# 86885974647565434342125458569795756674/torch.distributed.pipeline.sync.Pipe

Measured on AMD Instinct MI355X. Metric: tokens/sec for 12-layer Transformer at PP=N (pipeline-parallel training), higher is better.
Workload: dtype bf16

## Files before the change

mipipe/csrc/kernels/gemm.hip:

```cpp
#include <algorithm>
#include <cstdlib>
#include <type_traits>

#include "common.h"
#include "kernels.h"

namespace mipipe {

namespace {

constexpr int BM = 128, BN = 128, BK = 64;
constexpr int kThreads = 256;
constexpr int kTileBytes = BM * BK * 2;
constexpr int kBufBytes = 2 * kTileBytes;
constexpr int kSmemBytes = 2 * kBufBytes;

typedef __attribute__((ext_vector_type(4))) short s16x4;
typedef __attribute__((ext_vector_type(8))) short s16x8;
typedef __attribute__((address_space(3))) s16x4 lds_s16x4;

__device__ __forceinline__ int kc_off(int r, int c16) { return r * 128 + ((c16 ^ ((r >> 1) & 7)) << 4); }

__device__ __forceinline__ int ic_rk(int r) { return (r & 3) | (((r >> 3) & 1) << 2); }
__device__ __forceinline__ int ic_off(int r, int c8) { return r * 256 + ((c8 ^ (ic_rk(r) << 2)) << 3); }
// ... 72 lines not shown
}

template <bool A_KC, bool B_KC, int EPI, int ACT>
__global__ void __launch_bounds__(kThreads) gemm_kernel(GemmArgs g) {
  extern __shared__ __attribute__((aligned(16))) char smem[];
  const int tid = threadIdx.x;
  const int lane = tid & 63;
  const int wave = tid >> 6;
  const int wm = wave >> 1, wn = wave & 1;

  int tm, tn;
  tile_coords(g.M / BM, g.N / BN, tm, tn);
  const int m0 = tm * BM, n0 = tn * BN;

  const bf16_t* A = reinterpret_cast<const bf16_t*>(g.A);
  const bf16_t* B = reinterpret_cast<const bf16_t*>(g.B);

  f32x4 acc[4][4];
#pragma unroll
  for (int i = 0; i < 4; ++i)
#pragma unroll
    for (int j = 0; j < 4; ++j) acc[i][j] = f32x4{0.f, 0.f, 0.f, 0.f};

  Stager<A_KC> sa;
  Stager<B_KC> sb;
  const int nk = g.K / BK;

  sa.load(A, g.lda, m0, 0, tid);
  sb.load(B, g.ldb, n0, 0, tid);
  sa.store(smem, tid);
  sb.store(smem + kTileBytes, tid);
  __syncthreads();

  for (int kt = 0; kt < nk; ++kt) {
    char* cur = smem + (kt & 1) * kBufBytes;
    const bool more = kt + 1 < nk;
    if (more) {
      sa.load(A, g.lda, m0, (kt + 1) * BK, tid);
      sb.load(B, g.ldb, n0, (kt + 1) * BK, tid);
    }
#pragma unroll
    for (int s = 0; s < 2; ++s) {
      bf16x8 af[4], bfr[4];
#pragma unroll
      for (int t = 0; t < 4; ++t) af[t] = read_frag<A_KC>(cur, wm * 64 + 16 * t, s, lane);
#pragma unroll
      for (int t = 0; t < 4; ++t) bfr[t] = read_frag<B_KC>(cur + kTileBytes, wn * 64 + 16 * t, s, lane);
#pragma unroll
      for (int i = 0; i < 4; ++i)
#pragma unroll
        for (int j = 0; j < 4; ++j) acc[i][j] = __builtin_amdgcn_mfma_f32_16x16x32_bf16(af[i], bfr[j], acc[i][j], 0, 0, 0);
    }
    if (more) {
      char* nxt = smem + ((kt + 1) & 1) * kBufBytes;
      sa.store(nxt, tid);
      sb.store(nxt + kTileBytes, tid);
    }
    __syncthreads();
  }

  const int quad = lane >> 4, col_in = lane & 15;
  const float pscale = g.p > 0.f ? 1.f / (1.f - g.p) : 1.f;
#pragma unroll
  for (int i = 0; i < 4; ++i) {
    const int row0 = m0 + wm * 64 + 16 * i + 4 * quad;
#pragma unroll
    for (int j = 0; j < 4; ++j) {
      const int col = n0 + wn * 64 + 16 * j + col_in;
      f32x4 v = acc[i][j];
      if (EPI == kEpiAccumF32) {
        float* C = reinterpret_cast<float*>(g.C);
#pragma unroll
        for (int r = 0; r < 4; ++r) {
          float* p = C + (int64_t)(row0 + r) * g.ldc + col;
          *p += v[r];
        }
      } else if (EPI == kEpiStoreF32) {
        float* C = reinterpret_cast<float*>(g.C);
#pragma unroll
        for (int r = 0; r < 4; ++r) C[(int64_t)(row0 + r) * g.ldc + col] = v[r];
      } else {
        bf16_t* C = reinterpret_cast<bf16_t*>(g.C);
        const float b = g.bias != nullptr ? bf2f(reinterpret_cast<const bf16_t*>(g.bias)[col]) : 0.f;
        float pre[4], out[4];
#pragma unroll
        for (int r = 0; r < 4; ++r) {
          pre[r] = v[r] + b;
          out[r] = ACT == kActRelu ? fmaxf(pre[r], 0.f) : (ACT == kActGelu ? gelu_f(pre[r]) : pre[r]);
        }
        if (g.p > 0.f) {
          const uint4 w = Philox(g.seed, drop_sub(row0, col, g.N), g.offset).next4();
          const uint32_t ws[4] = {w.x, w.y, w.z, w.w};
#pragma unroll
          for (int r = 0; r < 4; ++r) out[r] = drop_keep(ws[r], col & 1, g.threshold >> 16) ? out[r] * pscale : 0.f;
        }
#pragma unroll
        for (int r = 0; r < 4; ++r) {
          if (g.dact_in != nullptr && g.dact == kActReluBits)
            out[r] *= (reinterpret_cast<const uint8_t*>(g.dact_in)[(int64_t)(row0 + r) * g.ldd + (col >> 3)] >> (col & 7)) & 1
                          ? g.dact_scale : 0.f;
          else if (g.dact_in != nullptr)
            out[r] *= g.dact_scale *
                      dact_f(g.dact, bf2f(reinterpret_cast<const bf16_t*>(g.dact_in)[(int64_t)(row0 + r) * g.ldd + col]));
          if (g.res != nullptr) out[r] += bf2f(reinterpret_cast<const bf16_t*>(g.res)[(int64_t)(row0 + r) * g.ldr + col]);
          C[(int64_t)(row0 + r) * g.ldc + col] = f2bf(out[r]);
          if (g.aux != nullptr)
            reinterpret_cast<bf16_t*>(g.aux)[(int64_t)(row0 + r) * g.ldc + col] =
                f2bf(g.aux_grad ? gelu_grad_f(pre[r]) : pre[r]);
        }
      }
    }
  }
}

namespace big {

constexpr int BM = 256, BN = 256, BK = 64;
constexpr int kThreads = 512;
constexpr int kTileBytes = BM * BK * 2;
constexpr int kSmemBytes = 128 * 260 * 4;

template <bool B_KC, int W>
constexpr int smem_bytes() {
  constexpr int b3 = 2 * (kTileBytes + W * BK * 2) + W * BK * 2;
  return !B_KC && b3 > kSmemBytes ? b3 : kSmemBytes;
}

template <int W>
__device__ __forceinline__ int ic_off_w(int r, int c8) { return r * (2 * W) + ((c8 ^ (ic_rk(r) << 2)) << 3); }

template <bool KC, int W>
__device__ __forceinline__ void stage_offsets(int64_t ld, int i0, int lim, int wave, int lane, uint32_t (&off)[W / 64]) {
  constexpr int NU = W / 64, LPR = W / 8;
#pragma unroll
  for (int u = 0; u < NU; ++u) {
    const int inst = wave * NU + u;
    if (KC) {
      const int row = 8 * inst + (lane >> 3);
      const int c = (lane & 7) ^ ((row >> 1) & 7);
      const int gi = min(i0 + row, lim - 1);
      off[u] = (uint32_t)(((int64_t)gi * ld + 8 * c) * 2);
    } else {
      const int row = (64 / LPR) * inst + lane / LPR;
      const int c16 = (lane % LPR) ^ (ic_rk(row) << 1);
      const int gi = min(i0 + 8 * c16, lim - 8);
      off[u] = (uint32_t)(((int64_t)row * ld + gi) * 2);
    }
  }
}

__device__ __forceinline__ void stage_offsets_halves(int64_t ld, int i0, int lim, int share, int lane,
                                                     uint32_t (&off)[4]) {
  const int half = share >> 2;
#pragma unroll
  for (int u = 0; u < 4; ++u) {
    const int row = 4 * (4 * (share & 3) + u) + (lane >> 4);
    const int c16 = (lane & 15) ^ (ic_rk(row) << 1);
    const int gi = min(i0 + 128 * half + 8 * c16, lim - 8);
    off[u] = (uint32_t)(((int64_t)row * ld + gi) * 2);
  }
}

__device__ __forceinline__ void glds16_saddr(const char* base, uint32_t off, const char* lds_dst) {
  const uint32_t m0 = (uint32_t)(uintptr_t)((__attribute__((address_space(3))) const char*)lds_dst);
  asm volatile(
      "s_mov_b32 m0, %0\n\t"
      "s_nop 0\n\t"
      "global_load_lds_dwordx4 %1, %2"
      :
      : "s"(m0), "v"(off), "s"(base)
      : "memory", "m0");
}

template <int N>
__device__ __forceinline__ void vmcnt_keep() {
  asm volatile("s_waitcnt vmcnt(%0)" ::"n"(N) : "memory");
}

constexpr int kWaitLgkm0 = 0xC07F;

template <int W>
__device__ __forceinline__ void stage_fast(const char* base, const uint32_t (&off)[W / 64], char* tile, int wave) {
  constexpr int NU = W / 64;
#pragma unroll
  for (int u = 0; u < NU; ++u) glds16_saddr(base, off[u], tile + (wave * NU + u) * 1024);
}

struct KCursor {
  const char *a, *b;
  const char *na, *nb;
  int64_t step_a, step_b;
  int seg_k, kl, seg;

  __device__ __forceinline__ void load_next(const GemmArgs& g) {
    const int nx = min(seg + 1, GemmArgs::kMaxSegs - 1);
    na = reinterpret_cast<const char*>(g.a_seg[nx]);
    nb = reinterpret_cast<const char*>(g.b_seg[nx]);
  }
  template <bool A_KC, bool B_KC>
  __device__ __forceinline__ void init(const GemmArgs& g, int kt) {
    const int64_t lda = g.lda, ldb = g.ldb;
    step_a = A_KC ? BK * 2 : BK * lda * 2;
    step_b = B_KC ? BK * 2 : BK * ldb * 2;
    seg_k = g.seg_k;
    kl = kt * BK;
    seg = 0;
    a = na = reinterpret_cast<const char*>(g.A);
    b = nb = reinterpret_cast<const char*>(g.B);
    if (seg_k > 0) {
      seg = kl / seg_k;
      kl -= seg * seg_k;
      a = reinterpret_cast<const char*>(g.a_seg[seg]);
      b = reinterpret_cast<const char*>(g.b_seg[seg]);
      load_next(g);
    }
    a += A_KC ? (int64_t)kl * 2 : (int64_t)kl * lda * 2;
    b += B_KC ? (int64_t)kl * 2 : (int64_t)kl * ldb * 2;
  }
  __device__ __forceinline__ void next(const GemmArgs& g) {
    a += step_a;
    b += step_b;
    kl += BK;
    if (__builtin_expect(kl == seg_k, 0)) {
      kl = 0;
      ++seg;
      a = na;
      b = nb;
      load_next(g);
    }
  }
};

template <bool KC, int W>
__device__ __forceinline__ bf16x8 frag(const char* tile, int ib, int s, int lane) {
  if (KC) {
    const int r = ib + (lane & 15);
    const int c = 4 * s + (lane >> 4);
    return *reinterpret_cast<const bf16x8*>(tile + kc_off(r, c));
  } else {
    const int g = lane >> 4, q = (lane & 15) >> 2, p = lane & 3;
    const int r0 = 32 * s + 8 * g + q;
    const int c8 = (ib >> 2) + p;
    const s16x4 lo = __builtin_amdgcn_ds_read_tr16_b64_v4i16((lds_s16x4*)(tile + ic_off_w<W>(r0, c8)));
    const s16x4 hi = __builtin_amdgcn_ds_read_tr16_b64_v4i16((lds_s16x4*)(tile + ic_off_w<W>(r0 + 4, c8)));
    return __builtin_bit_cast(bf16x8, __builtin_shufflevector(lo, hi, 0, 1, 2, 3, 4, 5, 6, 7));
  }
}

template <int W>
__device__ __forceinline__ uint32_t ic_frag_off(int ib, int lane) {
  const int g = lane >> 4, q = (lane & 15) >> 2, p = lane & 3;
  return (uint32_t)ic_off_w<W>(8 * g + q, (ib >> 2) + p);
}

template <int W>
__device__ __forceinline__ bf16x8 ic_frag_at(uint32_t addr, int imm, int s) {
  const s16x4 lo = __builtin_amdgcn_ds_read_tr16_b64_v4i16((lds_s16x4*)(addr + (uint32_t)(imm + s * 32 * 2 * W)));
  const s16x4 hi =
      __builtin_amdgcn_ds_read_tr16_b64_v4i16((lds_s16x4*)(addr + (uint32_t)(imm + s * 32 * 2 * W + 4 * 2 * W)));
  return __builtin_bit_cast(bf16x8, __builtin_shufflevector(lo, hi, 0, 1, 2, 3, 4, 5, 6, 7));
}

struct EpiParams {
  uint64_t seed, offset;
  int N;
  float p, pscale;
  uint32_t threshold;
  int mask_row0, mask_col0, mask_ld;
};

template <int I, int ACT, int NJ, bool EXTRA>
__device__ __forceinline__ void epi_rows(const EpiParams ep, f32x4 (&acc)[8][NJ], int nrow, int ncol,
                                         const float (&bias)[NJ]) {
  if constexpr (!EXTRA) {
#pragma unroll
    for (int j = 0; j < NJ; ++j)
#pragma unroll
      for (int r = 0; r < 4; ++r) {
        const float pre = acc[I][j][r] + bias[j];
        acc[I][j][r] = ACT == kActRelu ? fmaxf(pre, 0.f) : (ACT == kActGelu ? gelu_f(pre) : pre);
      }
    return;
  }
  const int row0 = nrow + 16 * I;
#pragma unroll
  for (int j = 0; j < NJ; ++j) {
    const int col = ncol + 16 * j;
    const float b = bias[j];
    uint32_t ws[4] = {0xFFFFFFFFu, 0xFFFFFFFFu, 0xFFFFFFFFu, 0xFFFFFFFFu};
    if (ep.p > 0.f) {
      const uint4 w = Philox(ep.seed, drop_sub(row0 + ep.mask_row0, col + ep.mask_col0, ep.mask_ld), ep.offset).next4();
      ws[0] = w.x; ws[1] = w.y; ws[2] = w.z; ws[3] = w.w;
    }
#pragma unroll
    for (int r = 0; r < 4; ++r) {
      const float pre = acc[I][j][r] + b;
      float out = ACT == kActRelu ? fmaxf(pre, 0.f) : (ACT == kActGelu ? gelu_f(pre) : pre);
      if (ep.p > 0.f) out = drop_keep(ws[r], (col + ep.mask_col0) & 1, ep.threshold >> 16) ? out * ep.pscale : 0.f;
      acc[I][j][r] = out;
    }
  }
}

template <int EPI, int W>
__device__ __forceinline__ void staged_store(char* smem, const f32x4 (&acc)[8][W / 64], int wm, int wn, int lane,
                                             int tid, int m0, int n0, int M, int N, int64_t ldc, void* out,
                                             const bf16_t* res, int64_t ldr = 0, const bf16_t* dact_in = nullptr,
                                             int64_t ldd = 0, int dact = 0, float dact_scale = 1.f,
                                             bool trans = false, bool dgelu = false) {
  constexpr int NJ = W / 64, WN = 16 * NJ, kStride = W + 4;
  const int quad = lane >> 4, col_in = lane & 15;
  float* stg = reinterpret_cast<float*>(smem);
#pragma unroll
  for (int pass = 0; pass < 2; ++pass) {
    if (wm == pass) {
#pragma unroll
      for (int i = 0; i < 8; ++i)
#pragma unroll
        for (int j = 0; j < NJ; ++j)
#pragma unroll
          for (int r = 0; r < 4; ++r)
            stg[(16 * i + 4 * quad + r) * kStride + wn * WN + 16 * j + col_in] = acc[i][j][r];
    }
    __syncthreads();
    const int rbase = m0 + pass * 128;
    auto grow = [&](int R) { return rbase + R; };
    if (EPI == kEpiStoreBf16) {
      bf16_t* C = reinterpret_cast<bf16_t*>(out);
      constexpr int CPR = W / 8;
#pragma unroll
      for (int u = 0; u < 128 * CPR / kThreads; ++u) {
        const int idx = tid + u * kThreads;
        const int row = idx / CPR, c8 = idx % CPR;
        if (grow(row) >= M || n0 + 8 * c8 >= N) continue;
        const f32x4 lo = *reinterpret_cast<const f32x4*>(stg + row * kStride + 8 * c8);
        const f32x4 hi = *reinterpret_cast<const f32x4*>(stg + row * kStride + 8 * c8 + 4);
        const int64_t at = (int64_t)grow(row) * ldc + n0 + 8 * c8;
        float v[8] = {lo[0], lo[1], lo[2], lo[3], hi[0], hi[1], hi[2], hi[3]};
        if (dgelu) {
#pragma unroll
          for (int e = 0; e < 8; ++e) v[e] = gelu_grad_f(v[e]);
        }
        if (dact_in != nullptr && dact == kActReluBits) {
          const uint32_t mb =
              reinterpret_cast<const uint8_t*>(dact_in)[(int64_t)grow(row) * ldd + ((n0 + 8 * c8) >> 3)];
#pragma unroll
          for (int e = 0; e < 8; ++e) v[e] *= (mb >> e) & 1 ? dact_scale : 0.f;
        } else if (dact_in != nullptr) {
          const bf16x8 sv = *reinterpret_cast<const bf16x8*>(dact_in + (int64_t)grow(row) * ldd + n0 + 8 * c8);
#pragma unroll
          for (int e = 0; e < 8; ++e) v[e] *= dact_scale * dact_f(dact, (float)sv[e]);
        }
        if (res != nullptr) {
          const bf16x8 rv = *reinterpret_cast<const bf16x8*>(res + (int64_t)grow(row) * ldr + n0 + 8 * c8);
#pragma unroll
          for (int e = 0; e < 8; ++e) v[e] += (float)rv[e];
        }
        bf16x8 o;
#pragma unroll
        for (int e = 0; e < 8; ++e) o[e] = (__bf16)v[e];
        *reinterpret_cast<bf16x8*>(C + at) = o;
      }
    } else if (trans) {
      float* C = reinterpret_cast<float*>(out);
#pragma unroll 4
      for (int u = 0; u < 32 * W / kThreads; ++u) {
        const int idx = tid + u * kThreads;
        const int mq = (idx & 7) + 8 * (idx / (8 * W)), n = (idx >> 3) % W;
        if (grow(4 * mq) >= M || n0 + n >= N) continue;
        const float* sp = stg + 4 * mq * kStride + n;
        const float4 v = make_float4(sp[0], sp[kStride], sp[2 * kStride], sp[3 * kStride]);
        float4* dst = reinterpret_cast<float4*>(C + (int64_t)(n0 + n) * ldc + grow(4 * mq));
        if (EPI == kEpiAccumF32) {
          const float4 o = *dst;
          *dst = make_float4(o.x + v.x, o.y + v.y, o.z + v.z, o.w + v.w);
        } else {
          *dst = v;
        }
      }
    } else {
      float* C = reinterpret_cast<float*>(out);
      constexpr int CPR = W / 4;
#pragma unroll
      for (int u = 0; u < 128 * CPR / kThreads; ++u) {
        const int idx = tid + u * kThreads;
        const int row = idx / CPR, c4 = idx % CPR;
        if (grow(row) >= M || n0 + 4 * c4 >= N) continue;
        const float4 v = *reinterpret_cast<const float4*>(stg + row * kStride + 4 * c4);
        float4* dst = reinterpret_cast<float4*>(C + (int64_t)grow(row) * ldc + n0 + 4 * c4);
        if (EPI == kEpiAccumF32) {
          const float4 o = *dst;
          *dst = make_float4(o.x + v.x, o.y + v.y, o.z + v.z, o.w + v.w);
        } else {
          *dst = v;
        }
      }
    }
    __syncthreads();
  }
}

template <int ACT, int W>
__device__ __forceinline__ void staged_store_act(char* smem, const f32x4 (&acc)[8][W / 64], int wm, int wn,
                                                 int lane, int tid, int m0, int n0, const GemmArgs& g) {
  constexpr int NJ = W / 64, WN = 16 * NJ, kStride = W + 4, CB = W / 8;
  const int quad = lane >> 4, col_in = lane & 15;
  float* stg = reinterpret_cast<float*>(smem);
  bf16_t* C = reinterpret_cast<bf16_t*>(g.C);
  bf16_t* aux = reinterpret_cast<bf16_t*>(g.aux);
  const bf16_t* res = reinterpret_cast<const bf16_t*>(g.res);
  const bf16_t* dact_in = reinterpret_cast<const bf16_t*>(g.dact_in);
  const int64_t ldr = g.ldr > 0 ? g.ldr : g.ldc;
  const bool drop = g.p > 0.f;
  const float pscale = drop ? 1.f / (1.f - g.p) : 1.f;
  const int64_t mask_ld = g.mask_ld > 0 ? g.mask_ld : g.N;
  const uint32_t thr16 = g.threshold >> 16;
#pragma unroll
  for (int pass = 0; pass < 2; ++pass) {
    if (wm == pass) {
#pragma unroll
      for (int i = 0; i < 8; ++i)
#pragma unroll
        for (int j = 0; j < NJ; ++j)
#pragma unroll
          for (int r = 0; r < 4; ++r)
            stg[(16 * i + 4 * quad + r) * kStride + wn * WN + 16 * j + col_in] = acc[i][j][r];
    }
    __syncthreads();
    const int rbase = m0 + pass * 128;
#pragma unroll
    for (int u = 0; u < 32 * CB / kThreads; ++u) {
      const int idx = tid + u * kThreads;
      const int rq = idx / CB, c8 = idx % CB;
      const int col = n0 + 8 * c8;
      const int row0 = rbase + 4 * rq;
      if (col >= g.N || row0 >= g.M) continue;
      uint32_t wd[4][4];
      if (drop) {
        const uint64_t sub = drop_sub(row0 + g.mask_row0, col + g.mask_col0, mask_ld);
#pragma unroll
        for (int e = 0; e < 4; ++e) {
          const uint4 w = Philox(g.seed, sub + e, g.offset).next4();
          wd[e][0] = w.x; wd[e][1] = w.y; wd[e][2] = w.z; wd[e][3] = w.w;
        }
      }
#pragma unroll
      for (int r = 0; r < 4; ++r) {
        const int row = row0 + r;
        if (row >= g.M) break;
        const float* sp = stg + (4 * rq + r) * kStride + 8 * c8;
        const f32x4 lo = *reinterpret_cast<const f32x4*>(sp);
        const f32x4 hi = *reinterpret_cast<const f32x4*>(sp + 4);
        const float pre[8] = {lo[0], lo[1], lo[2], lo[3], hi[0], hi[1], hi[2], hi[3]};
        if (aux != nullptr) {
          bf16x8 a;
#pragma unroll
          for (int e = 0; e < 8; ++e) a[e] = (__bf16)(ACT == kActGelu && g.aux_grad ? gelu_grad_f(pre[e]) : pre[e]);
          *reinterpret_cast<bf16x8*>(aux + (int64_t)row * g.ldc + col) = a;
        }
        float v[8];
#pragma unroll
        for (int e = 0; e < 8; ++e) {
          float o = ACT == kActRelu ? fmaxf(pre[e], 0.f) : (ACT == kActGelu ? gelu_f(pre[e]) : pre[e]);
          if (drop) o = drop_keep(wd[e >> 1][r], e & 1, thr16) ? o * pscale : 0.f;
          v[e] = o;
        }
        if (dact_in != nullptr) {
          const bf16x8 sv = *reinterpret_cast<const bf16x8*>(dact_in + (int64_t)row * g.ldd + col);
#pragma unroll
          for (int e = 0; e < 8; ++e) v[e] *= g.dact_scale * dact_f(g.dact, (float)sv[e]);
        }
        if (res != nullptr) {
          const bf16x8 rv = *reinterpret_cast<const bf16x8*>(res + (int64_t)row * ldr + col);
#pragma unroll
          for (int e = 0; e < 8; ++e) v[e] += (float)rv[e];
        }
        bf16x8 o;
#pragma unroll
        for (int e = 0; e < 8; ++e) o[e] = (__bf16)v[e];
        *reinterpret_cast<bf16x8*>(C + (int64_t)row * g.ldc + col) = o;
        if (g.bits != nullptr) {
          uint32_t mb = 0;
#pragma unroll
          for (int e = 0; e < 8; ++e) mb |= (v[e] != 0.f ? 1u : 0u) << e;
          reinterpret_cast<uint8_t*>(g.bits)[(int64_t)row * g.ldbits + (col >> 3)] = (uint8_t)mb;
        }
      }
    }
    __syncthreads();
  }
}


constexpr int kXEmit = 1, kXColsum = 2;

template <bool A_KC, bool B_KC, int EPI, int ACT, int W, bool EXTRA, int X = 0>
__global__ void __launch_bounds__(kThreads, 1) gemm256_kernel(GemmArgs g) {
  constexpr int NJ = W / 64;
  constexpr int WN = W / 4;
  constexpr int kBuf = kTileBytes + W * BK * 2;
  constexpr bool AH = !A_KC;
  constexpr bool B3 = !B_KC;
  constexpr bool II = AH && B3;
  extern __shared__ __attribute__((aligned(16))) char smem[];
  const int tid = threadIdx.x;
  const int lane = tid & 63;
  const int wave = __builtin_amdgcn_readfirstlane(tid >> 6);
  const int wm = wave >> 2, wn = wave & 3;

  int tm, tn;
  tile_coords((g.M + BM - 1) / BM, (g.N + W - 1) / W, tm, tn, g.group_m);
  tm = __builtin_amdgcn_readfirstlane(tm);
  tn = __builtin_amdgcn_readfirstlane(tn);
  const int m0 = tm * BM, n0 = tn * W;
  f32x4 acc[8][NJ];
#pragma unroll
  for (int i = 0; i < 8; ++i)
#pragma unroll
    for (int j = 0; j < NJ; ++j) acc[i][j] = f32x4{0.f, 0.f, 0.f, 0.f};

  const bool rsum = g.rowsum != nullptr && tn < 16 && !A_KC;
  float rs[4] = {0.f, 0.f, 0.f, 0.f};
  auto rowsum_read = [&](const char* tile, s16x4& v) {
    if (rsum && wm == 0) {
      const int r = tid >> 2, c8 = 4 * tn + (tid & 3);
      v = *reinterpret_cast<const s16x4*>(
          AH ? tile + (tn >> 3) * (kTileBytes / 2) + ic_off_w<128>(r, c8 & 31) : tile + ic_off_w<256>(r, c8));
    }
  };
  auto rowsum_add = [&](const s16x4& v) {
    if (rsum && wm == 0) {
#pragma unroll
      for (int e = 0; e < 4; ++e) rs[e] += __uint_as_float((uint32_t)(uint16_t)v[e] << 16);
    }
  };
  const int tiles_m = (g.M + BM - 1) / BM;
  const int cm_log = __builtin_amdgcn_readfirstlane(2 * tiles_m * 16 >= W ? 0 : 2 * tiles_m * 32 >= W ? 1
                                                    : 2 * tiles_m * 64 >= W ? 2 : 3);
  const int csl = tm + tiles_m * wm;
  const bool csum = X == kXColsum && !B_KC && g.colsum != nullptr && csl < (W / 16 >> cm_log);
  float cs[4] = {0.f, 0.f, 0.f, 0.f};
  auto colsum_step = [&](const char* btile) {
    if (csum) {
      const int t = tid & 255;
      const int q = t & ((4 << cm_log) - 1), r0 = t >> (2 + cm_log);
      for (int j = 0; j < (1 << cm_log); ++j) {
        const s16x4 v = *reinterpret_cast<const s16x4*>(
            btile + ic_off_w<W>(r0 + (j << (6 - cm_log)), (4 << cm_log) * csl + q));
#pragma unroll
        for (int e = 0; e < 4; ++e) cs[e] += __uint_as_float((uint32_t)(uint16_t)v[e] << 16);
      }
    }
  };
  const int ntn = (g.N + W - 1) / W;
  const int ewb = __builtin_amdgcn_readfirstlane((4 * wave) % ntn);
  auto emit_reads = [&](const char* atile, int j, s16x4& a, s16x4& b) {
    const int q = (lane & 15) >> 2, p = lane & 3, gq = lane >> 4;
    const int c16 = 2 * gq + (p >> 1);
    const int r = 8 * (4 * wave + j) + q;
    const int lo = r * 128 + ((c16 ^ ((r >> 1) & 7)) << 4) + 8 * (p & 1);
    const int hi = (r + 4) * 128 + ((c16 ^ (((r + 4) >> 1) & 7)) << 4) + 8 * (p & 1);
    a = __builtin_amdgcn_ds_read_tr16_b64_v4i16((lds_s16x4*)(atile + lo));
    b = __builtin_amdgcn_ds_read_tr16_b64_v4i16((lds_s16x4*)(atile + hi));
  };
  bf16_t* const at_out = X == kXEmit ? reinterpret_cast<bf16_t*>(g.at) : nullptr;
  const int64_t ldat = X == kXEmit ? g.ldat : 0;
  const int M = g.M;
  auto emit_store = [&](int kt, int j, const s16x4& a, const s16x4& b) {
    const int rb = 4 * wave + j;
    bf16_t* at = at_out + (int64_t)(kt * BK + 16 * (lane >> 4) + (lane & 15)) * ldat + m0 + 8 * rb;
    if (m0 + 8 * rb < M) *reinterpret_cast<s16x8*>(at) = __builtin_shufflevector(a, b, 0, 1, 2, 3, 4, 5, 6, 7);
  };
  int kt0 = 0, nk = g.K / BK;
  if (g.k_splits > 1) {
    const int total = nk;
    kt0 = (int)blockIdx.y * total / g.k_splits;
    nk = ((int)blockIdx.y + 1) * total / g.k_splits - kt0;
  }
  const int shA = wave ^ 4;
  const int shB = B_KC ? 2 * wn + (wm == 0 ? 1 : 0) : wave;
  uint32_t offA[4], offB[NJ];
  if constexpr (AH) stage_offsets_halves(g.lda, m0, g.M, shA, lane, offA);
  else stage_offsets<A_KC, 256>(g.lda, m0, g.M, shA, lane, offA);
  stage_offsets<B_KC, W>(g.ldb, n0, g.N, shB, lane, offB);
  constexpr int NB = W / 64;
  constexpr int NA = 4;
  auto abuf = [&](int i) { return II ? smem + i * kTileBytes : smem + i * kBuf; };
  auto bslot = [&](int s) {
    if (II) return smem + 2 * kTileBytes + s * (W * BK * 2);
    return s == 2 ? smem + 2 * kBuf : smem + s * kBuf + kTileBytes;
  };
  KCursor kc;
  kc.init<A_KC, B_KC>(g, kt0);
  stage_fast<256>(kc.a, offA, abuf(0), shA);
  stage_fast<W>(kc.b, offB, bslot(0), shB);
  kc.next(g);
  if (wm == 1 && nk > 1) {
    stage_fast<256>(kc.a, offA, abuf(1), shA);
    stage_fast<W>(kc.b, offB, bslot(1), shB);
    kc.next(g);
  }

  if (wm == 1 && nk > 1) vmcnt_keep<NA + NB>();
  else asm volatile("s_waitcnt vmcnt(0)" ::: "memory");
  __builtin_amdgcn_s_barrier();
  if (wm == 1) __builtin_amdgcn_s_barrier();
  bf16x8 af[8][2], bq[NJ][2];
  int ekt = kt0 % ntn;
  int bs = 0;
  if constexpr (II) {
    const uint32_t lds0 = (uint32_t)(uintptr_t)((__attribute__((address_space(3))) const char*)smem);
    uint32_t aaddr[8], baddr[NJ];
#pragma unroll
    for (int ii = 0; ii < 8; ++ii) aaddr[ii] = lds0 + wm * (kTileBytes / 2) + ic_frag_off<128>(16 * ii, lane);
#pragma unroll
    for (int j = 0; j < NJ; ++j) baddr[j] = ic_frag_off<W>(wn * WN + 16 * j, lane);
    auto k_tile = [&](const int u, auto parity) {
      constexpr int P = decltype(parity)::value;
      char* cur = abuf(P);
      char* nxt = abuf(P ^ 1);
      char* bcur = bslot(bs);
#pragma unroll
      for (int ii = 0; ii < 8; ++ii)
#pragma unroll
        for (int s = 0; s < 2; ++s) af[ii][s] = ic_frag_at<128>(aaddr[ii], P * kTileBytes, s);
      const uint32_t bcur0 = (uint32_t)(uintptr_t)((__attribute__((address_space(3))) const char*)bcur);
#pragma unroll
      for (int j = 0; j < NJ; ++j) {
        const uint32_t ba = bcur0 + baddr[j];
#pragma unroll
        for (int s = 0; s < 2; ++s) bq[j][s] = ic_frag_at<W>(ba, 0, s);
      }
      s16x4 rv;
      rowsum_read(cur, rv);
      const int ahead = wm == 0 ? 1 : 2;
      if (u + ahead < nk) {
        stage_fast<256>(kc.a, offA, wm == 0 ? nxt : cur, shA);
        int bn = bs + ahead;
        if (bn >= 3) bn -= 3;
        stage_fast<W>(kc.b, offB, bslot(bn), shB);
        kc.next(g);
      }
      bs = bs == 2 ? 0 : bs + 1;
      if (wm == 1) {
        if (u + 2 < nk) vmcnt_keep<NA + NB>();
        else asm volatile("s_waitcnt vmcnt(0)" ::: "memory");
      }
      __builtin_amdgcn_s_waitcnt(kWaitLgkm0);
      rowsum_add(rv);
      __builtin_amdgcn_sched_barrier(0);
      __builtin_amdgcn_s_barrier();
      __builtin_amdgcn_sched_barrier(0);
      __builtin_amdgcn_s_setprio(1);
#pragma unroll
      for (int s = 0; s < 2; ++s)
#pragma unroll
        for (int ii = 0; ii < 8; ++ii)
#pragma unroll
          for (int j = 0; j < NJ; ++j)
            acc[ii][j] = __builtin_amdgcn_mfma_f32_16x16x32_bf16(af[ii][s], bq[j][s], acc[ii][j], 0, 0, 0);
      __builtin_amdgcn_s_setprio(0);
      if (wm == 0) asm volatile("s_waitcnt vmcnt(0)" ::: "memory");
      __builtin_amdgcn_sched_barrier(0);
      __builtin_amdgcn_s_barrier();
      __builtin_amdgcn_sched_barrier(0);
    };
    for (int u = 0; u < nk; u += 2) {
      k_tile(u, std::integral_constant<int, 0>{});
      if (u + 1 < nk) k_tile(u + 1, std::integral_constant<int, 1>{});
    }
  }
  for (int u = 0; !II && u < nk; ++u) {
    char* cur = smem + (u & 1) * kBuf;
    char* nxt = smem + ((u + 1) & 1) * kBuf;
    char* bcur = B3 ? bslot(bs) : cur + kTileBytes;
    int ej = -1;
    if (X == kXEmit && A_KC) {
      int e = ewb + ekt;
      while (e >= ntn) e -= ntn;
      ej = tn - e;
      if (ej < 0) ej += ntn;
      if (ntn < 4) {
        for (int j = ej; j < 4; j += ntn) {
          s16x4 a, b;
          emit_reads(cur, j, a, b);
          emit_store(kt0 + u, j, a, b);
        }
        ej = -1;
      } else if (ej > 3) {
        ej = -1;
      }
    }
    s16x4 ea, eb;
    if (X == kXEmit && A_KC && ej >= 0) emit_reads(cur, ej, ea, eb);
#pragma unroll
    for (int ii = 0; ii < 8; ++ii)
#pragma unroll
      for (int s = 0; s < 2; ++s)
        af[ii][s] = AH ? frag<false, 128>(cur + wm * (kTileBytes / 2), 16 * ii, s, lane)
                       : frag<A_KC, 256>(cur, wm * 128 + 16 * ii, s, lane);
#pragma unroll
    for (int j = 0; j < NJ; ++j)
#pragma unroll
      for (int s = 0; s < 2; ++s) bq[j][s] = frag<B_KC, W>(bcur, wn * WN + 16 * j, s, lane);
    s16x4 rv;
    rowsum_read(cur, rv);
    if (X == kXEmit && A_KC && ej >= 0) emit_store(kt0 + u, ej, ea, eb);
    ekt = ekt + 1 == ntn ? 0 : ekt + 1;
    const int ahead = wm == 0 ? 1 : 2;
    if (u + ahead < nk) {
      char* dst = wm == 0 ? nxt : cur;
      stage_fast<256>(kc.a, offA, dst, shA);
      int bn = bs + ahead;
      if (bn >= 3) bn -= 3;
      stage_fast<W>(kc.b, offB, B3 ? bslot(bn) : dst + kTileBytes, shB);
      kc.next(g);
    }
    bs = bs == 2 ? 0 : bs + 1;
    colsum_step(bcur);
    if (wm == 1) {
      if (u + 2 < nk) vmcnt_keep<NA + NB>();
      else asm volatile("s_waitcnt vmcnt(0)" ::: "memory");
    }
    __builtin_amdgcn_s_waitcnt(kWaitLgkm0);
    rowsum_add(rv);
    __builtin_amdgcn_sched_barrier(0);
    __builtin_amdgcn_s_barrier();
    __builtin_amdgcn_sched_barrier(0);
    __builtin_amdgcn_s_setprio(1);
#pragma unroll
    for (int s = 0; s < 2; ++s)
#pragma unroll
      for (int ii = 0; ii < 8; ++ii)
#pragma unroll
        for (int j = 0; j < NJ; ++j)
          acc[ii][j] = __builtin_amdgcn_mfma_f32_16x16x32_bf16(af[ii][s], bq[j][s], acc[ii][j], 0, 0, 0);
    __builtin_amdgcn_s_setprio(0);
    if (wm == 0) asm volatile("s_waitcnt vmcnt(0)" ::: "memory");
    __builtin_amdgcn_sched_barrier(0);
    __builtin_amdgcn_s_barrier();
    __builtin_amdgcn_sched_barrier(0);
  }
  if (wm == 0) __builtin_amdgcn_s_barrier();

  if (rsum) {
    __syncthreads();
    float* red = reinterpret_cast<float*>(smem);
    if (wm == 0) {
#pragma unroll
      for (int e = 0; e < 4; ++e)
#pragma unroll
        for (int o = 4; o < 64; o <<= 1) rs[e] += __shfl_xor(rs[e], o, 64);
      if (lane < 4)
#pragma unroll
        for (int e = 0; e < 4; ++e) red[wave * 16 + 4 * lane + e] = rs[e];
    }
    __syncthreads();
    if (tid < 16) {
      const float v = red[tid] + red[16 + tid] + red[32 + tid] + red[48 + tid];
      const int row = m0 + 16 * tn + tid;
      if (row < g.M) g.rowsum[row] += v;
    }
  }
  if (X == kXColsum && g.colsum != nullptr) {
    __syncthreads();
    const int sw = 16 << cm_log;
    float* red = reinterpret_cast<float*>(smem) + 64;
#pragma unroll
    for (int e = 0; e < 4; ++e)
      for (int o = 4 << cm_log; o < 64; o <<= 1) cs[e] += __shfl_xor(cs[e], o, 64);
    if (lane < (4 << cm_log))
#pragma unroll
      for (int e = 0; e < 4; ++e) red[wave * sw + 4 * lane + e] = cs[e];
    __syncthreads();
    if (tid < 2 * sw) {
      const int gq = tid >> (4 + cm_log), c = tid & (sw - 1);
      const int sl = tm + tiles_m * gq;
      float v = 0.f;
#pragma unroll
      for (int w = 0; w < 4; ++w) v += red[(4 * gq + w) * sw + c];
      const int col = n0 + sw * sl + c;
      if (sl < (W / 16 >> cm_log) && col < g.N) {
        if (g.k_splits > 1) g.colsum[(int64_t)blockIdx.y * g.N + col] = v;
        else g.colsum[col] += v;
      }
    }
  }
  const int quad = lane >> 4, col_in = lane & 15;
  __syncthreads();
  if (EPI == kEpiStoreBf16 && EXTRA) {
    const int ncol = n0 + wn * WN + col_in;
    if (g.bias != nullptr) {
#pragma unroll
      for (int j = 0; j < NJ; ++j) {
        const float b = ncol + 16 * j < g.N ? bf2f(reinterpret_cast<const bf16_t*>(g.bias)[ncol + 16 * j]) : 0.f;
#pragma unroll
        for (int i = 0; i < 8; ++i) acc[i][j] += b;
      }
    }
    staged_store_act<ACT, W>(smem, acc, wm, wn, lane, tid, m0, n0, g);
    return;
  }
  if (EPI == kEpiStoreBf16 && (ACT != kActNone || g.bias != nullptr)) {
    const int ncol = n0 + wn * WN + col_in, nrow = m0 + wm * 128 + 4 * quad;
    const float pscale = g.p > 0.f ? 1.f / (1.f - g.p) : 1.f;
    const EpiParams ep{g.seed, g.offset, g.N, g.p, pscale, g.threshold, g.mask_row0, g.mask_col0,
                       g.mask_ld > 0 ? g.mask_ld : g.N};
    float bias[NJ];
#pragma unroll
    for (int j = 0; j < NJ; ++j)
      bias[j] = (g.bias != nullptr && ncol + 16 * j < g.N) ? bf2f(reinterpret_cast<const bf16_t*>(g.bias)[ncol + 16 * j]) : 0.f;
    epi_rows<0, ACT, NJ, EXTRA>(ep, acc, nrow, ncol, bias);
    epi_rows<1, ACT, NJ, EXTRA>(ep, acc, nrow, ncol, bias);
    epi_rows<2, ACT, NJ, EXTRA>(ep, acc, nrow, ncol, bias);
    epi_rows<3, ACT, NJ, EXTRA>(ep, acc, nrow, ncol, bias);
    epi_rows<4, ACT, NJ, EXTRA>(ep, acc, nrow, ncol, bias);
    epi_rows<5, ACT, NJ, EXTRA>(ep, acc, nrow, ncol, bias);
    epi_rows<6, ACT, NJ, EXTRA>(ep, acc, nrow, ncol, bias);
    epi_rows<7, ACT, NJ, EXTRA>(ep, acc, nrow, ncol, bias);
  }
  void* out = EPI == kEpiStoreBf16 ? g.C
                                   : reinterpret_cast<void*>(reinterpret_cast<float*>(g.C) +
                                                             (int64_t)blockIdx.y * g.M * g.ldc);
  if (EPI == kEpiStoreBf16 && g.dact_in != nullptr)
    staged_store<EPI, W>(smem, acc, wm, wn, lane, tid, m0, n0, g.M, g.N, g.ldc, out,
                         reinterpret_cast<const bf16_t*>(g.res), g.ldr, reinterpret_cast<const bf16_t*>(g.dact_in),
                         g.ldd, g.dact, g.dact_scale);
  else if (EPI != kEpiStoreBf16 && g.trans_c && g.k_splits <= 1)
    staged_store<EPI, W>(smem, acc, wm, wn, lane, tid, m0, n0, g.M, g.N, g.ldc, out, nullptr, 0, nullptr, 0, 0, 1.f,
                         true);
  else
    staged_store<EPI, W>(smem, acc, wm, wn, lane, tid, m0, n0, g.M, g.N, g.ldc, out,
                         EPI == kEpiStoreBf16 ? reinterpret_cast<const bf16_t*>(g.res) : nullptr, g.ldr);
}

}

int big_tiles(const GemmArgs& g, int w) { return ((g.M + big::BM - 1) / big::BM) * ((g.N + w - 1) / w); }

bool use_big(const GemmArgs& g) {
  return g.round_chunk || g.seg_k > 0 || g.at != nullptr || g.trans_c || g.colsum != nullptr || g.rowsum != nullptr ||
         g.M % BM != 0 || g.N % BN != 0 || big_tiles(g, 256) >= 128;
}

int g_gemm_width = -1;
int g_gemm_rounds = -1;

int big_width(const GemmArgs& g) {
  if (g_gemm_width < 0) {
    const char* e = getenv("MIPIPE_GEMM_W");
    g_gemm_width = e ? atoi(e) : 0;
  }
  if (g_gemm_width == 128 || g_gemm_width == 256) return g_gemm_width;
  if (g.width == 128 || g.width == 256) return g.width;
  if (g.k_splits > 1) return 256;
  const int r256 = (big_tiles(g, 256) + 255) / 256, r128 = (big_tiles(g, 128) + 255) / 256;
  return 0.75 * r128 < 1.0 * r256 ? 128 : 256;
}

template <bool A_KC, bool B_KC, int EPI, int ACT, int W, bool EXTRA, int X = 0>
void launch_big(const GemmArgs& g, hipStream_t s) {
  constexpr int smem = big::smem_bytes<B_KC, W>();
  static bool attr_set = false;
  if (!attr_set) {
    (void)hipFuncSetAttribute(
        reinterpret_cast<const void*>(&big::gemm256_kernel<A_KC, B_KC, EPI, ACT, W, EXTRA, X>),
        hipFuncAttributeMaxDynamicSharedMemorySize, smem);
    attr_set = true;
  }
  hipLaunchKernelGGL((big::gemm256_kernel<A_KC, B_KC, EPI, ACT, W, EXTRA, X>), dim3(big_tiles(g, W), g.k_splits),
                     dim3(big::kThreads), smem, s, g);
}

template <bool A_KC, bool B_KC, int EPI, int ACT, bool EXTRA>
void launch_big_w(const GemmArgs& g, hipStream_t s) {
  const bool narrow = big_width(g) == 128;
  if constexpr (A_KC && B_KC && EPI == kEpiStoreBf16 && !(ACT == kActGelu && EXTRA)) {
    if (g.at != nullptr) {
      if (narrow) launch_big<A_KC, B_KC, EPI, ACT, 128, EXTRA, big::kXEmit>(g, s);
      else launch_big<A_KC, B_KC, EPI, ACT, 256, EXTRA, big::kXEmit>(g, s);
      return;
    }
  }
  if constexpr (A_KC && !B_KC && EPI != kEpiStoreBf16 && !EXTRA) {
    if (g.colsum != nullptr) {
      if (narrow) launch_big<A_KC, B_KC, EPI, ACT, 128, EXTRA, big::kXColsum>(g, s);
      else launch_big<A_KC, B_KC, EPI, ACT, 256, EXTRA, big::kXColsum>(g, s);
      return;
    }
  }
  if (narrow) launch_big<A_KC, B_KC, EPI, ACT, 128, EXTRA>(g, s);
  else launch_big<A_KC, B_KC, EPI, ACT, 256, EXTRA>(g, s);
}

int g_gemm_group = -1;

template <bool A_KC, bool B_KC, int EPI, int ACT>
void launch(const GemmArgs& gi, hipStream_t s) {
  if (g_gemm_group < 0) {
    const char* e = getenv("MIPIPE_GEMM_G");
    g_gemm_group = e ? atoi(e) : 0;
  }
  GemmArgs g = gi;
  if (g_gemm_group > 0) g.group_m = g_gemm_group;
  if (use_big(g)) {
    if constexpr (EPI == kEpiStoreBf16) {
      if (g.p > 0.f || g.aux != nullptr) {
        launch_big_w<A_KC, B_KC, EPI, ACT, true>(g, s);
        return;
      }
    }
    launch_big_w<A_KC, B_KC, EPI, ACT, false>(g, s);
    return;
  }
  const int blocks = (g.M / BM) * (g.N / BN);
  hipLaunchKernelGGL((gemm_kernel<A_KC, B_KC, EPI, ACT>), dim3(blocks), dim3(kThreads), kSmemBytes, s, g);
}

__global__ void __launch_bounds__(256) splitk_reduce_kernel(const float* __restrict__ ws, int splits, int M, int N,
                                                            int64_t ldc, const bf16_t* __restrict__ res, int64_t ldr,
                                                            bf16_t* __restrict__ C) {
  const int64_t chunks = (int64_t)M * (N / 8);
  const int64_t c = (int64_t)blockIdx.x * blockDim.x + threadIdx.x;
  if (c >= chunks) return;
  const int row = (int)(c / (N / 8)), col = (int)(c % (N / 8)) * 8;
  const int64_t at = (int64_t)row * N + col;
  f32x4 lo = *reinterpret_cast<const f32x4*>(ws + at);
  f32x4 hi = *reinterpret_cast<const f32x4*>(ws + at + 4);
  for (int s = 1; s < splits; ++s) {
    lo += *reinterpret_cast<const f32x4*>(ws + (int64_t)s * M * N + at);
    hi += *reinterpret_cast<const f32x4*>(ws + (int64_t)s * M * N + at + 4);
  }
  float v[8] = {lo[0], lo[1], lo[2], lo[3], hi[0], hi[1], hi[2], hi[3]};
  const int64_t out = (int64_t)row * ldc + col;
  if (res != nullptr) {
    const bf16x8 r = *reinterpret_cast<const bf16x8*>(res + (int64_t)row * ldr + col);
#pragma unroll
    for (int e = 0; e < 8; ++e) v[e] += (float)r[e];
  }
  bf16x8 o;
#pragma unroll
  for (int e = 0; e < 8; ++e) o[e] = (__bf16)v[e];
  *reinterpret_cast<bf16x8*>(C + out) = o;
}

__global__ void __launch_bounds__(256) splitk_reduce_f32_kernel(const float* __restrict__ ws, int splits, int M, int N,
                                                                int64_t ldc, bool accumulate, bool trans,
                                                                float* __restrict__ C) {
  const int64_t c = (int64_t)blockIdx.x * blockDim.x + threadIdx.x;
  if (trans) {
    if (c >= (int64_t)(M / 4) * N) return;
    const int m = (int)(c / N) * 4, n = (int)(c % N);
    f32x4 v = {0.f, 0.f, 0.f, 0.f};
    for (int s = 0; s < splits; ++s) {
      const float* p = ws + (int64_t)s * M * N + (int64_t)m * N + n;
      v += f32x4{p[0], p[N], p[2 * (int64_t)N], p[3 * (int64_t)N]};
    }
    f32x4* dst = reinterpret_cast<f32x4*>(C + (int64_t)n * ldc + m);
    if (accumulate) v += *dst;
    *dst = v;
    return;
  }
  const int64_t chunks = (int64_t)M * (N / 4);
  if (c >= chunks) return;
  const int row = (int)(c / (N / 4)), col = (int)(c % (N / 4)) * 4;
  const int64_t at = (int64_t)row * N + col;
  f32x4 v = *reinterpret_cast<const f32x4*>(ws + at);
  for (int s = 1; s < splits; ++s) v += *reinterpret_cast<const f32x4*>(ws + (int64_t)s * M * N + at);
  f32x4* dst = reinterpret_cast<f32x4*>(C + (int64_t)row * ldc + col);
  if (accumulate) v += *dst;
  *dst = v;
}

__global__ void __launch_bounds__(256) colsum_splits_kernel(const float* __restrict__ ws, int splits, int N,
                                                            float* __restrict__ colsum) {
  const int n = blockIdx.x * blockDim.x + threadIdx.x;
  if (n >= N) return;
  float v = 0.f;
  for (int s = 0; s < splits; ++s) v += ws[(int64_t)s * N + n];
  colsum[n] += v;
}

int g_gemm_splitk = -1;

template <bool A_KC, bool B_KC, int EPI>
void launch_act(const GemmArgs& g, hipStream_t s) {
  switch (g.act) {
    case kActRelu: launch<A_KC, B_KC, EPI, kActRelu>(g, s); break;
    case kActGelu: launch<A_KC, B_KC, EPI, kActGelu>(g, s); break;
    default: launch<A_KC, B_KC, EPI, kActNone>(g, s); break;
  }
}

}

void gemm_set_width(int w) { g_gemm_width = w; }
void gemm_set_rounds(int on) { g_gemm_rounds = on; }
void gemm_set_splitk(int n) { g_gemm_splitk = n; }

bool gemm_rowsum_ok(const GemmArgs& g) {
  return !g.a_kc && (g.epi == kEpiAccumF32 || g.epi == kEpiStoreF32) && use_big(g) && gemm_splitk_factor(g) <= 1 &&
         (g.N + big_width(g) - 1) / big_width(g) >= 16;
}

bool gemm_bits_ok(const GemmArgs& g) {
  return g.epi == kEpiStoreBf16 && g.act == kActRelu && g.p > 0.f && g.k_splits <= 1 && g.N % 8 == 0 && use_big(g);
}

bool gemm_emit_ok(int act, float p, bool aux) { return !(act == kActGelu && (p > 0.f || aux)); }

bool gemm_colsum_ok(const GemmArgs& g) {
  if (g.b_kc || !g.a_kc || !(g.epi == kEpiAccumF32 || g.epi == kEpiStoreF32)) return false;
  GemmArgs b = g;
  b.k_splits = gemm_splitk_factor(g);
  const int w = big_width(b);
  return 2 * ((g.M + big::BM - 1) / big::BM) * 128 >= w;
}

bool gemm_supported(int64_t M, int64_t N, int64_t K) {
  return M >= 8 && N >= 8 && K > 0 && M % 8 == 0 && N % 8 == 0 && K % BK == 0 && M < (1LL << 30) &&
         N < (1LL << 30) && M * K < (1LL << 31) && N * K < (1LL << 31);
}

int gemm_splitk_factor(const GemmArgs& g) {
  if (g_gemm_splitk < 0) {
    const char* e = getenv("MIPIPE_GEMM_SPLITK");
    g_gemm_splitk = e ? atoi(e) : 1;
  }
  if (g_gemm_splitk == 0) return 1;
  const bool plain_bf16 = g.epi == kEpiStoreBf16 && g.act == kActNone && g.bias == nullptr && g.p <= 0.f &&
                          g.aux == nullptr && g.dact_in == nullptr;
  const bool f32_out = g.epi == kEpiAccumF32 || g.epi == kEpiStoreF32;
  if (!(plain_bf16 || f32_out) || !use_big(g) || g.K < 8192) return 1;
  const int tiles = big_tiles(g, 256);
  const int kt = g.K / BK;
  if (g_gemm_splitk >= 2) return std::max(1, std::min(g_gemm_splitk, kt / 16));
  const double t_tile = 2.0 * 256 * 256 * (double)g.K / 4.5e12;
  const double mn = (double)g.M * g.N;
  int best = 1;
  double best_t = (double)((tiles + 255) / 256) * t_tile;
  for (int sp = 2; sp <= 8 && kt / sp >= 16; ++sp) {
    const double t = (double)((tiles * sp + 255) / 256) * t_tile / sp + (2.0 * sp + 1.0) * 4.0 * mn / 4.0e12;
    if (t < 0.97 * best_t) {
      best = sp;
      best_t = t;
    }
  }
  return best;
}


static const char* byte_off(const void* p, int64_t bytes) {
  return p == nullptr ? nullptr : reinterpret_cast<const char*>(p) + bytes;
}

template <typename F>
bool launch_by_rounds(const GemmArgs& g, F&& run) {
  if (g_gemm_rounds < 0) {
    const char* e = getenv("MIPIPE_GEMM_ROUNDS");
    g_gemm_rounds = e ? atoi(e) : 1;
  }
  if (g_gemm_rounds == 0 || g.k_splits > 1 || !use_big(g) || big_width(g) != 256) return false;
  if (g_gemm_rounds == 1 && g.K < 4096) return false;
  const int tm = (g.M + 255) / 256, tn = (g.N + 255) / 256;
  if (tm * tn <= 256 || (tm * tn) % 256 == 0 || (tm * tn) % 256 > 128) return false;
  const bool along_n = tn >= tm;
  if (along_n && g.rowsum != nullptr) return false;
  if (!along_n && g.colsum != nullptr) return false;
  const int other = along_n ? tm : tn, along = along_n ? tn : tm;
  const int per = 256 / other;
  if (per < 1 || (along + per - 1) / per > 16) return false;
  const int cbytes = g.epi == kEpiStoreBf16 ? 2 : 4;
  for (int t0 = 0; t0 < along; t0 += per) {
    GemmArgs c = g;
    c.round_chunk = true;
    c.width = 256;
    const int lo = t0 * 256, hi = std::min((t0 + per) * 256, along_n ? g.N : g.M);
    c.mask_ld = g.mask_ld > 0 ? g.mask_ld : g.N;
    if (along_n) {
      c.N = hi - lo;
      c.mask_col0 = g.mask_col0 + lo;
      const int64_t boff = (g.b_kc ? (int64_t)lo * g.ldb : (int64_t)lo) * 2;
      c.B = byte_off(g.B, boff);
      for (int i = 0; i < GemmArgs::kMaxSegs; ++i) c.b_seg[i] = byte_off(g.b_seg[i], boff);
      c.C = const_cast<char*>(byte_off(g.C, (g.trans_c ? (int64_t)lo * g.ldc : (int64_t)lo) * cbytes));
      if (g.colsum != nullptr) c.colsum = g.colsum + lo;
      if (t0 > 0) c.at = nullptr;
      c.bias = byte_off(g.bias, (int64_t)lo * 2);
      c.aux = const_cast<char*>(byte_off(g.aux, (int64_t)lo * 2));
      c.res = byte_off(g.res, (int64_t)lo * 2);
      c.dact_in = byte_off(g.dact_in, g.dact == kActReluBits ? (int64_t)lo / 8 : (int64_t)lo * 2);
      c.bits = const_cast<char*>(byte_off(g.bits, (int64_t)lo / 8));
    } else {
      c.M = hi - lo;
      c.mask_row0 = g.mask_row0 + lo;
      if (g.rowsum != nullptr) c.rowsum = g.rowsum + lo;
      const int64_t aoff = (g.a_kc ? (int64_t)lo * g.lda : (int64_t)lo) * 2;
      c.A = byte_off(g.A, aoff);
      for (int i = 0; i < GemmArgs::kMaxSegs; ++i) c.a_seg[i] = byte_off(g.a_seg[i], aoff);
      c.C = const_cast<char*>(byte_off(g.C, (g.trans_c ? (int64_t)lo : (int64_t)lo * g.ldc) * cbytes));
      c.at = const_cast<char*>(byte_off(g.at, (int64_t)lo * 2));
      c.aux = const_cast<char*>(byte_off(g.aux, (int64_t)lo * g.ldc * 2));
      c.res = byte_off(g.res, (int64_t)lo * g.ldr * 2);
      c.dact_in = byte_off(g.dact_in, (int64_t)lo * g.ldd * (g.dact == kActReluBits ? 1 : 2));
      c.bits = const_cast<char*>(byte_off(g.bits, (int64_t)lo * g.ldbits));
    }
    run(c);
  }
  return true;
}

void gemm_bf16(const GemmArgs& gi, hipStream_t s) {
  GemmArgs g = gi;
  g.threshold = dropout_threshold(g.p);
  if (g.ldr == 0) g.ldr = g.ldc;
  if (g.ldd == 0) g.ldd = g.ldc;
  if (g.k_splits > 1) {
    GemmArgs p = g;
    p.epi = kEpiStoreF32;
    p.C = g.ws;
    p.ldc = g.N;
    p.res = nullptr;
    p.trans_c = false;
    p.rowsum = nullptr;
    p.colsum = g.colsum != nullptr ? g.colsum_ws : nullptr;
    if (p.a_kc && p.b_kc) launch<true, true, kEpiStoreF32, kActNone>(p, s);
    else if (p.a_kc && !p.b_kc) launch<true, false, kEpiStoreF32, kActNone>(p, s);
    else if (!p.a_kc && !p.b_kc) launch<false, false, kEpiStoreF32, kActNone>(p, s);
    else launch<false, true, kEpiStoreF32, kActNone>(p, s);
    if (g.epi == kEpiStoreBf16) {
      const int64_t chunks = (int64_t)g.M * (g.N / 8);
      hipLaunchKernelGGL(splitk_reduce_kernel, dim3((unsigned)((chunks + 255) / 256)), dim3(256), 0, s, g.ws,
                         g.k_splits, g.M, g.N, g.ldc, reinterpret_cast<const bf16_t*>(g.res), g.ldr,
                         reinterpret_cast<bf16_t*>(g.C));
    } else {
      const int64_t chunks = (int64_t)g.M * (g.N / 4);
// ... 32 lines not shown
```

Measured before the change: 152,800.

## Prefetch residual and activation side inputs in GEMM epilogue, specialize store paths

Specializes the bf16 staged-store epilogue by side-input type (none, residual, relu bits, activation, both) and by whether the tile touches a matrix edge. For residual-only or bits-only cases it issues the global loads for both passes before the LDS staging and barrier, so their latency overlaps the accumulator spill. The activation-fused store loads residual and activation rows ahead of the dropout and activation math. Edge handling uses clamped addresses, and interior tiles skip the bounds checks. In exchange the templates hold more registers (side-input arrays kept across passes), there are more kernel instantiations, and the unused dgelu parameter is removed.

Result: no change. 154,100, median of 6 (+0.9%).

```diff
diff --git a/mipipe/csrc/kernels/gemm.hip b/mipipe/csrc/kernels/gemm.hip
--- a/mipipe/csrc/kernels/gemm.hip
+++ b/mipipe/csrc/kernels/gemm.hip
@@ -398,15 +398,48 @@
   }
 }
 
-template <int EPI, int W>
+constexpr int kSideNone = 0, kSideRes = 1, kSideBits = 2, kSideAct = 3, kSideAny = 4;
+
+template <int EPI, int W, int SIDE = kSideNone, bool EDGE = true>
 __device__ __forceinline__ void staged_store(char* smem, const f32x4 (&acc)[8][W / 64], int wm, int wn, int lane,
                                              int tid, int m0, int n0, int M, int N, int64_t ldc, void* out,
                                              const bf16_t* res, int64_t ldr = 0, const bf16_t* dact_in = nullptr,
                                              int64_t ldd = 0, int dact = 0, float dact_scale = 1.f,
-                                             bool trans = false, bool dgelu = false) {
+                                             bool trans = false) {
   constexpr int NJ = W / 64, WN = 16 * NJ, kStride = W + 4;
+  constexpr int CPR = W / 8, NU = 128 * CPR / kThreads, RS = kThreads / CPR;
+  constexpr bool kAhead = SIDE == kSideRes || SIDE == kSideBits;
+  constexpr int NB = SIDE == kSideAny && NU > 4 ? NU / 2 : NU;
   const int quad = lane >> 4, col_in = lane & 15;
   float* stg = reinterpret_cast<float*>(smem);
+  const int row_t = tid / CPR, col = n0 + 8 * (tid % CPR);
+  u32x4 rv[2][NU], sv[NU];
+  uint32_t mb[2][NU];
+  const bool bits = SIDE == kSideBits || (SIDE == kSideAny && dact == kActReluBits);
+  auto fetch = [&](int pass, int b) {
+    if (EPI != kEpiStoreBf16 || SIDE == kSideNone) return;
+    const int h = kAhead ? pass : 0;
+    const int row = m0 + pass * 128 + row_t;
+    auto at = [&](int u, int64_t ld, int shift) {
+      if (EDGE) return (int64_t)min(row + u * RS, M - 1) * ld + (min(col, N - 8) >> shift);
+      return (int64_t)row * ld + (col >> shift) + (int64_t)(u * RS) * ld;
+    };
+    if (SIDE == kSideRes || SIDE == kSideAny) {
+#pragma unroll
+      for (int u = b; u < b + NB; ++u) rv[h][u] = *reinterpret_cast<const u32x4*>(res + at(u, ldr, 0));
+    }
+    if (bits) {
+#pragma unroll
+      for (int u = b; u < b + NB; ++u) mb[h][u] = reinterpret_cast<const uint8_t*>(dact_in)[at(u, ldd, 3)];
+    } else if (SIDE == kSideAct || SIDE == kSideAny) {
+#pragma unroll
+      for (int u = b; u < b + NB; ++u) sv[u] = *reinterpret_cast<const u32x4*>(dact_in + at(u, ldd, 0));
+    }
+  };
+  if (kAhead) {
+    fetch(0, 0);
+    fetch(1, 0);
+  }
 #pragma unroll
   for (int pass = 0; pass < 2; ++pass) {
     if (wm == pass) {
@@ -418,44 +451,39 @@
           for (int r = 0; r < 4; ++r)
             stg[(16 * i + 4 * quad + r) * kStride + wn * WN + 16 * j + col_in] = acc[i][j][r];
     }
+    if (!kAhead) fetch(pass, 0);
     __syncthreads();
     const int rbase = m0 + pass * 128;
     auto grow = [&](int R) { return rbase + R; };
     if (EPI == kEpiStoreBf16) {
-      bf16_t* C = reinterpret_cast<bf16_t*>(out);
-      constexpr int CPR = W / 8;
-#pragma unroll
-      for (int u = 0; u < 128 * CPR / kThreads; ++u) {
-        const int idx = tid + u * kThreads;
-        const int row = idx / CPR, c8 = idx % CPR;
-        if (grow(row) >= M || n0 + 8 * c8 >= N) continue;
-        const f32x4 lo = *reinterpret_cast<const f32x4*>(stg + row * kStride + 8 * c8);
-        const f32x4 hi = *reinterpret_cast<const f32x4*>(stg + row * kStride + 8 * c8 + 4);
-        const int64_t at = (int64_t)grow(row) * ldc + n0 + 8 * c8;
-        float v[8] = {lo[0], lo[1], lo[2], lo[3], hi[0], hi[1], hi[2], hi[3]};
-        if (dgelu) {
-#pragma unroll
-          for (int e = 0; e < 8; ++e) v[e] = gelu_grad_f(v[e]);
+      bf16_t* C = reinterpret_cast<bf16_t*>(out) + (int64_t)grow(row_t) * ldc + col;
+      const int h = kAhead ? pass : 0;
+#pragma unroll
+      for (int u = 0; u < NU; ++u) {
+        if (u == NB) fetch(pass, NB);
+        const int row = row_t + u * RS;
+        if (!EDGE || (grow(row) < M && col < N)) {
+          const f32x4 lo = *reinterpret_cast<const f32x4*>(stg + row * kStride + (col - n0));
+          const f32x4 hi = *reinterpret_cast<const f32x4*>(stg + row * kStride + (col - n0) + 4);
+          float v[8] = {lo[0], lo[1], lo[2], lo[3], hi[0], hi[1], hi[2], hi[3]};
+          if (bits) {
+#pragma unroll
+            for (int e = 0; e < 8; ++e) v[e] *= (mb[h][u] >> e) & 1 ? dact_scale : 0.f;
+          } else if (SIDE == kSideAct || SIDE == kSideAny) {
+            const bf16x8 s8 = __builtin_bit_cast(bf16x8, sv[u]);
+#pragma unroll
+            for (int e = 0; e < 8; ++e) v[e] *= dact_scale * dact_f(dact, (float)s8[e]);
+          }
+          if (SIDE == kSideRes || SIDE == kSideAny) {
+            const bf16x8 r8 = __builtin_bit_cast(bf16x8, rv[h][u]);
+#pragma unroll
+            for (int e = 0; e < 8; ++e) v[e] += (float)r8[e];
+          }
+          bf16x8 o;
+#pragma unroll
+          for (int e = 0; e < 8; ++e) o[e] = (__bf16)v[e];
+          *reinterpret_cast<bf16x8*>(C + (int64_t)(u * RS) * ldc) = o;
         }
-        if (dact_in != nullptr && dact == kActReluBits) {
-          const uint32_t mb =
-              reinterpret_cast<const uint8_t*>(dact_in)[(int64_t)grow(row) * ldd + ((n0 + 8 * c8) >> 3)];
-#pragma unroll
-          for (int e = 0; e < 8; ++e) v[e] *= (mb >> e) & 1 ? dact_scale : 0.f;
-        } else if (dact_in != nullptr) {
-          const bf16x8 sv = *reinterpret_cast<const bf16x8*>(dact_in + (int64_t)grow(row) * ldd + n0 + 8 * c8);
-#pragma unroll
-          for (int e = 0; e < 8; ++e) v[e] *= dact_scale * dact_f(dact, (float)sv[e]);
-        }
-        if (res != nullptr) {
-          const bf16x8 rv = *reinterpret_cast<const bf16x8*>(res + (int64_t)grow(row) * ldr + n0 + 8 * c8);
-#pragma unroll
-          for (int e = 0; e < 8; ++e) v[e] += (float)rv[e];
-        }
-        bf16x8 o;
-#pragma unroll
-        for (int e = 0; e < 8; ++e) o[e] = (__bf16)v[e];
-        *reinterpret_cast<bf16x8*>(C + at) = o;
       }
     } else if (trans) {
       float* C = reinterpret_cast<float*>(out);
@@ -500,13 +528,15 @@
 __device__ __forceinline__ void staged_store_act(char* smem, const f32x4 (&acc)[8][W / 64], int wm, int wn,
                                                  int lane, int tid, int m0, int n0, const GemmArgs& g) {
   constexpr int NJ = W / 64, WN = 16 * NJ, kStride = W + 4, CB = W / 8;
+  constexpr int NB = 32 * CB / kThreads;
   const int quad = lane >> 4, col_in = lane & 15;
   float* stg = reinterpret_cast<float*>(smem);
   bf16_t* C = reinterpret_cast<bf16_t*>(g.C);
   bf16_t* aux = reinterpret_cast<bf16_t*>(g.aux);
   const bf16_t* res = reinterpret_cast<const bf16_t*>(g.res);
   const bf16_t* dact_in = reinterpret_cast<const bf16_t*>(g.dact_in);
-  const int64_t ldr = g.ldr > 0 ? g.ldr : g.ldc;
+  const int64_t ldr = g.ldr > 0 ? g.ldr : g.ldc, ldd = g.ldd;
+  const int M = g.M, colc = min(n0 + 8 * (tid % CB), g.N - 8);
   const bool drop = g.p > 0.f;
   const float pscale = drop ? 1.f / (1.f - g.p) : 1.f;
   const int64_t mask_ld = g.mask_ld > 0 ? g.mask_ld : g.N;
@@ -525,11 +555,22 @@
     __syncthreads();
     const int rbase = m0 + pass * 128;
 #pragma unroll
-    for (int u = 0; u < 32 * CB / kThreads; ++u) {
+    for (int u = 0; u < NB; ++u) {
       const int idx = tid + u * kThreads;
       const int rq = idx / CB, c8 = idx % CB;
       const int col = n0 + 8 * c8;
       const int row0 = rbase + 4 * rq;
+      u32x4 rv[4], sv[4];
+      if (res != nullptr) {
+#pragma unroll
+        for (int r = 0; r < 4; ++r)
+          rv[r] = *reinterpret_cast<const u32x4*>(res + (int64_t)min(row0 + r, M - 1) * ldr + colc);
+      }
+      if (dact_in != nullptr) {
+#pragma unroll
+        for (int r = 0; r < 4; ++r)
+          sv[r] = *reinterpret_cast<const u32x4*>(dact_in + (int64_t)min(row0 + r, M - 1) * ldd + colc);
+      }
       if (col >= g.N || row0 >= g.M) continue;
       uint32_t wd[4][4];
       if (drop) {
@@ -562,14 +603,14 @@
           v[e] = o;
         }
         if (dact_in != nullptr) {
-          const bf16x8 sv = *reinterpret_cast<const bf16x8*>(dact_in + (int64_t)row * g.ldd + col);
-#pragma unroll
-          for (int e = 0; e < 8; ++e) v[e] *= g.dact_scale * dact_f(g.dact, (float)sv[e]);
+          const bf16x8 s8 = __builtin_bit_cast(bf16x8, sv[r]);
+#pragma unroll
+          for (int e = 0; e < 8; ++e) v[e] *= g.dact_scale * dact_f(g.dact, (float)s8[e]);
         }
         if (res != nullptr) {
-          const bf16x8 rv = *reinterpret_cast<const bf16x8*>(res + (int64_t)row * ldr + col);
-#pragma unroll
-          for (int e = 0; e < 8; ++e) v[e] += (float)rv[e];
+          const bf16x8 r8 = __builtin_bit_cast(bf16x8, rv[r]);
+#pragma unroll
+          for (int e = 0; e < 8; ++e) v[e] += (float)r8[e];
         }
         bf16x8 o;
 #pragma unroll
@@ -918,16 +959,38 @@
   void* out = EPI == kEpiStoreBf16 ? g.C
                                    : reinterpret_cast<void*>(reinterpret_cast<float*>(g.C) +
                                                              (int64_t)blockIdx.y * g.M * g.ldc);
-  if (EPI == kEpiStoreBf16 && g.dact_in != nullptr)
-    staged_store<EPI, W>(smem, acc, wm, wn, lane, tid, m0, n0, g.M, g.N, g.ldc, out,
-                         reinterpret_cast<const bf16_t*>(g.res), g.ldr, reinterpret_cast<const bf16_t*>(g.dact_in),
-                         g.ldd, g.dact, g.dact_scale);
-  else if (EPI != kEpiStoreBf16 && g.trans_c && g.k_splits <= 1)
+  if constexpr (EPI == kEpiStoreBf16) {
+    const bf16_t* res = reinterpret_cast<const bf16_t*>(g.res);
+    const bf16_t* dact_in = reinterpret_cast<const bf16_t*>(g.dact_in);
+    const int side = dact_in != nullptr
+                         ? (res != nullptr ? kSideAny : (g.dact == kActReluBits ? kSideBits : kSideAct))
+                         : (res != nullptr ? kSideRes : kSideNone);
+    const bool edge = m0 + BM > g.M || n0 + W > g.N;
+    const int lane_e = __builtin_amdgcn_mbcnt_hi(~0u, __builtin_amdgcn_mbcnt_lo(~0u, 0u));
+    const int tid_e = wave * 64 + lane_e;
+#define MIPIPE_STORE_BF16(SIDE, EDGE)                                                                          \
+  staged_store<EPI, W, SIDE, EDGE>(smem, acc, wm, wn, lane_e, tid_e, m0, n0, g.M, g.N, g.ldc, out, res, g.ldr, dact_in, \
+                                   g.ldd, g.dact, g.dact_scale)
+    if (edge) {
+      if (side == kSideNone) MIPIPE_STORE_BF16(kSideNone, true);
+      else if (side == kSideRes) MIPIPE_STORE_BF16(kSideRes, true);
+      else if (side == kSideBits) MIPIPE_STORE_BF16(kSideBits, true);
+      else if (side == kSideAct) MIPIPE_STORE_BF16(kSideAct, true);
+      else MIPIPE_STORE_BF16(kSideAny, true);
+    } else {
+      if (side == kSideNone) MIPIPE_STORE_BF16(kSideNone, false);
+      else if (side == kSideRes) MIPIPE_STORE_BF16(kSideRes, false);
+      else if (side == kSideBits) MIPIPE_STORE_BF16(kSideBits, false);
+      else if (side == kSideAct) MIPIPE_STORE_BF16(kSideAct, false);
+      else MIPIPE_STORE_BF16(kSideAny, false);
+    }
+#undef MIPIPE_STORE_BF16
+  } else if (g.trans_c && g.k_splits <= 1) {
     staged_store<EPI, W>(smem, acc, wm, wn, lane, tid, m0, n0, g.M, g.N, g.ldc, out, nullptr, 0, nullptr, 0, 0, 1.f,
                          true);
-  else
-    staged_store<EPI, W>(smem, acc, wm, wn, lane, tid, m0, n0, g.M, g.N, g.ldc, out,
-                         EPI == kEpiStoreBf16 ? reinterpret_cast<const bf16_t*>(g.res) : nullptr, g.ldr);
+  } else {
+    staged_store<EPI, W>(smem, acc, wm, wn, lane, tid, m0, n0, g.M, g.N, g.ldc, out, nullptr, g.ldr);
+  }
 }
 
 }
```
